# Mikata-Project/adcraft

Measured on AMD Instinct MI355X. Metric: env-steps/sec (envs×keywords auctions/s), higher is better.
Workload: dtype i32 cents + f32 (Philox4x32-7 u32); 1 GPU; cfg2: 4096 envs x 256 keywords per GPU, IMPLICIT keywords, mean_volume 128, cvr 0.8, no_vol_prob 0.0, drift False, budget non-binding, 60-step episodes with auto-reset; envs_per_gpu=4096, keywords=256, parallelism=env-sharded x1, collective=none (single GPU), weak_scaling_reference=also.cfg4.value of the N=1 --full line (same per-GPU shard as the N>1 runs)

## Files before the change

adcraft_amd/_ffi.py:

```python
import ctypes as C
import os

from . import build as _build

ADC_OK, ADC_EINVAL, ADC_EHIP, ADC_ENOMEM, ADC_ESTATE, ADC_ETYPE, ADC_ERCCL = 0, -1, -2, -3, -4, -5, -6
MODEL_IMPLICIT, MODEL_EXPLICIT, MODEL_IMPLICIT_GENERAL = 0, 1, 2
P_VOL_MEAN, P_VOL_STD, P_A, P_B, P_BCTR, P_SCTR, P_REV_MEAN, P_REV_STD, P_COUNT = range(9)
(BUF_PARAMS, BUF_BIDS, BUF_BUDGET, BUF_IMPRESSIONS, BUF_CLICKS, BUF_CONVERSIONS, BUF_COST, BUF_REVENUE, BUF_REWARD,
 BUF_CUM_PROFIT, BUF_DAYS, BUF_TERMINATED, BUF_TRUNCATED, BUF_METRIC_PROFIT, BUF_METRIC_SCALARS, BUF_FLAT_OBS,
 BUF_ROLLOUT_ACTION, BUF_ROLLOUT_LOGP, BUF_ROLLOUT_VALUE, BUF_ROLLOUT_REWARD, BUF_ROLLOUT_TERMINATED, BUF_ROLLOUT_TRUNCATED,
 BUF_ROLLOUT_OBS) = range(23)
MLP_TANH, MLP_RELU = 0, 1
ES_CENTERED_RANK, ES_RAW = 0, 1
ES_ADAM, ES_SGD = 0, 1
ROLLOUT_OBS = 1
PG_ADAM, PG_SGD = 0, 1
TD3_ADAM, TD3_SGD = 0, 1
PBT_PG, PBT_TD3 = 0, 1


class EngineError(RuntimeError):
    pass


# ... 194 lines not shown
        "adc_engine_metrics_reset": ([vp], C.c_int),
        "adc_engine_metrics_read": ([vp, vp, vp], C.c_int),
        "adc_engine_ideal_profit": ([vp, C.c_int, vp, C.c_int, vp], C.c_int),
        "adc_bid_curves_from_samples": ([C.c_int, vp, i32, vp, i32, vp, vp], C.c_int),
        "adc_engine_metrics_akncp_ncp": ([vp, f64, vp, vp], C.c_int),
        "adc_engine_bid_curves_contenders": ([vp, vp, vp, C.POINTER(i32)], C.c_int),
        "adc_engine_outcomes_replay": ([vp, i32, i32, vp, f32, i64, vp, vp, vp, vp, C.POINTER(i64), vp], C.c_int),
        "adc_engine_outcomes_replay_tape": ([vp, i32, vp, f32, C.POINTER(Tape), i64, vp, vp, vp, vp, C.POINTER(i64), vp], C.c_int),
        "adc_nth_price_auction": ([C.c_int, f64, vp, i32, i32, i32, i32, C.POINTER(i32), vp, vp], C.c_int),
        "adc_sigmoid": ([f64, f64, f64], f64),
        "adc_clamp": ([f64, f64, f64], f64),
        "adc_threshold_sigmoid": ([f64, f64, f64, f64], f64),
        "adc_sum_f64": ([vp, i64], f64),
        "adc_count_true": ([vp, i64], i64),
        "adc_nonneg_int_normal": ([f64, f64, u64, u64], u64),
        "adc_binomial": ([u64, f64, u64, u64], u64),
        "adc_cost_create": ([f64, i64, u64, u64, vp], C.c_int),
        "adc_auction_word_intervals": ([f32, f32, f32, f32, vp], C.c_int),
        "adc_auction_word_brackets": ([f32, f32, f32, f32, vp], C.c_int),
        "adc_check_win_brackets": ([i64, vp, vp, vp, vp, vp, vp, vp], i64),
        "adc_lower_bound_v_host": ([i64, vp, vp, vp, vp, vp], C.c_int),
        "adc_lower_bound_v_bisect_host": ([i64, vp, vp, vp, vp, vp], C.c_int),
        "adc_win_intervals_host": ([i64, vp, vp, vp, vp, i32, vp, vp], C.c_int),
        "adc_sample_random_keyword": ([C.c_uint64, C.c_uint32, C.c_uint32, vp], C.c_int),
        "adc_interp_act_host": ([f32, i32, f32, i32, C.c_double, C.c_double, C.c_double, vp, i32, i32, vp, vp, i32, vp, vp,
                                 C.c_double, vp, vp, vp, vp, vp], C.c_int),
        "adc_interp_key_host": ([f32], C.c_double),
        "adc_engine_mlp_init": ([vp, C.POINTER(MLPConfig), vp], C.c_int),
        "adc_engine_mlp_set_layer": ([vp, i32, i32, vp, vp], C.c_int),
        "adc_engine_mlp_set_norm": ([vp, vp, vp], C.c_int),
        "adc_engine_mlp_set_log_std": ([vp, vp], C.c_int),
        "adc_engine_mlp_set_deterministic": ([vp, i32], C.c_int),
        "adc_engine_mlp_act": ([vp, f32, vp], C.c_int),
        "adc_engine_mlp_step": ([vp, f32], C.c_int),
        "adc_engine_mlp_last": ([vp, vp, vp, vp, vp, vp], C.c_int),
        "adc_engine_mlp_bootstrap_value": ([vp, vp], C.c_int),
        "adc_engine_mlp_agent_state": ([vp, vp, vp], C.c_int),
        "adc_engine_rollout_enable": ([vp, i32, i32], C.c_int),
        "adc_engine_rollout_reset": ([vp], C.c_int),
        "adc_engine_rollout_fetch": ([vp, C.POINTER(i32), vp, vp, vp, vp, vp, vp, vp], C.c_int),
        "adc_engine_mlp_population": ([vp, i32, vp], C.c_int),
        "adc_engine_mlp_set_member_layer": ([vp, i32, i32, vp, vp], C.c_int),
        "adc_engine_mlp_param_count": ([vp, C.POINTER(i64)], C.c_int),
        "adc_engine_mlp_get_params": ([vp, vp], C.c_int),
        "adc_engine_mlp_get_member_params": ([vp, i32, vp], C.c_int),
        "adc_engine_mlp_learners": ([vp, i32], C.c_int),
# ... 171 lines not shown
```

adcraft_amd/build.py:

```python
import os
import subprocess
import sys

HERE = os.path.dirname(os.path.abspath(__file__))
ROOT = os.path.dirname(HERE)
SRC_DIR = os.path.join(HERE, "csrc")
LIB_DIR = os.path.join(HERE, "lib")
LIB = os.path.join(LIB_DIR, "libadcraft_hip.so")
SOURCES = ["adc_engine.hip", "adc_shims.cpp"]
HEADERS = ["adc_law.h", "adc_interp.h", "adc_mlp.h", "adc_es.h", "adc_pg.h", "adc_td3.h", "adc_pbt.h", "adc_norm.h", "adc_rew_norm.h", "adc_td3_norm.h", os.path.join(ROOT, "include", "adcraft_engine.h")] + sorted(
    os.path.join("parts", f) for f in os.listdir(os.path.join(SRC_DIR, "parts")) if f.endswith(".inc"))
HIPCC = os.environ.get("HIPCC", "/opt/rocm/bin/hipcc")
FLAGS = ["--offload-arch=gfx950", "-O3", "-std=c++17", "-fPIC", "-shared", "-fvisibility=hidden",
         "-ffp-contract=off", "-fno-fast-math", "-fhip-fp32-correctly-rounded-divide-sqrt",
         "-Wall", "-Wno-unused-function"]


def _deps():
    out = [os.path.join(SRC_DIR, s) for s in SOURCES]
    out += [h if os.path.isabs(h) else os.path.join(SRC_DIR, h) for h in HEADERS]
    return [p for p in out if os.path.exists(p)]


def source_hash():
    import hashlib
    h = hashlib.sha256()
    for p in sorted(_deps()):
        h.update(os.path.relpath(p, ROOT).encode() + b"\0")
        with open(p, "rb") as f:
            h.update(f.read())
    return h.hexdigest()[:16]


# ... 60 lines not shown
```

adcraft_amd/csrc/adc_engine.hip:

```cpp
#include <hip/hip_runtime.h>

#include <algorithm>
#include <chrono>
#include <type_traits>
#include <cmath>
#include <cstdio>
#include <cstdlib>
#include <cstring>
#include <new>
#include <string>
#include <vector>

#include "../../include/adcraft_engine.h"
#include "adc_law.h"
#include "adc_interp.h"
#include "adc_mlp.h"
#include "adc_es.h"
#include "adc_pg.h"
#include "adc_td3.h"
#include "adc_pbt.h"
#include "adc_norm.h"
#include "adc_rew_norm.h"
#include "adc_td3_norm.h"

#define ADC_EXPORT extern "C" __attribute__((visibility("default")))

namespace adck {
#include "parts/common.inc"
#include "parts/kernel_fast.inc"
#include "parts/kernel_sparse.inc"
#include "parts/kernel_exact_rows.inc"
#include "parts/kernel_click_walk.inc"
#include "parts/kernel_exact_serial.inc"
#include "parts/kernel_explicit_fast.inc"
#include "parts/kernels_misc.inc"
#include "parts/kernels_policy.inc"
#include "parts/kernel_explicit_curves.inc"
// ... 23 lines not shown
```

adcraft_amd/csrc/adc_shims.cpp:

```cpp
#include <algorithm>
#include <cmath>
#include <cstdint>
#include <thread>
#include <vector>

#include "../../include/adcraft_engine.h"
#include "adc_law.h"
#include "adc_interp.h"
#include "adc_mlp.h"
#include "adc_es.h"
#include "adc_pg.h"
#include "adc_td3.h"
#include "adc_pbt.h"
#include "adc_norm.h"
#include "adc_rew_norm.h"
#include "adc_td3_norm.h"

#define ADC_EXPORT extern "C" __attribute__((visibility("default")))

ADC_EXPORT double adc_sigmoid(double x, double s, double t) { return 1.0 / (1.0 + std::exp(-s * (x - t))); }

ADC_EXPORT double adc_clamp(double x, double lo, double hi) { return x < lo ? lo : (x > hi ? hi : x); }

ADC_EXPORT double adc_threshold_sigmoid(double p, double impression_thresh, double impression_bid_intercept,
                                        double impression_slope)
{
    const double halver = 2.0 + 1e-10;
    const double thresh = adc_clamp(halver * impression_thresh, 0.0, 1.0) / halver;
    const double r = adc_sigmoid(p, impression_slope, impression_bid_intercept);
    return adc_clamp((1.0 + 2.0 * thresh) * r - thresh, 0.0, 1.0);
// ... 161 lines not shown
    if (n < 0 || (n > 0 && (!bid_c || !cost_loc || !cost_scale || !buyside_ctr || !out4))) return ADC_EINVAL;
    const adc::LogTableEntry *table = host_log_table();
    shim_parallel_for(n, [=](int64_t i0, int64_t i1) {
        for (int64_t i = i0; i < i1; ++i) {
            const adc::AuctionLaw law = adc::make_auction_law(buyside_ctr[i]);
            const uint64_t t_click = adc::bernoulli_threshold(buyside_ctr[i]);
            uint32_t w_lo, w_hi;
            int stage = 0;
            if (bisect) {
                bool a = false, b = false;
                w_lo = adc::lower_bound_v_bisect(1 - bid_c[i], cost_loc[i], cost_scale[i], table, &a);
                w_hi = adc::lower_bound_v_bisect(bid_c[i], cost_loc[i], cost_scale[i], table, &b);
                stage = (a || b) ? 1 : 0;
            } else {
                adc::lower_bound_pair(bid_c[i], cost_loc[i], cost_scale[i], table, w_lo, w_hi, stage);
            }
            const adc::WinIntervals r = adc::win_intervals_of_bounds(w_lo, w_hi, t_click, law);
            uint32_t *o = out4 + 4 * i;
            o[0] = r.c_lo; o[1] = r.c_w; o[2] = r.n_lo; o[3] = r.n_w;
            if (stage_out) stage_out[i] = (uint8_t)stage;
        }
    });
    return ADC_OK;
}

ADC_EXPORT int adc_sample_random_keyword(uint64_t key, uint32_t keyword, uint32_t serial, float *out8)
{
    if (!out8) return ADC_EINVAL;
    adc::generate_explicit_keyword(key, keyword, serial, out8);
    return ADC_OK;
}

ADC_EXPORT int adc_explicit_curve_host(uint64_t key, uint32_t tick, int32_t keyword, int32_t n_samples, float impression_thresh, float a,
                                       float b, const double *bid_grid, int32_t n_bids, double *ir_out, double *cpc_out, double *z_mid2_out)
{
    if (n_samples <= 0 || n_samples > (1 << 20) || keyword < 0 || n_bids < 0 || (n_bids > 0 && (!bid_grid || !ir_out || !cpc_out)))
        return ADC_EINVAL;
    std::vector<float> z((size_t)n_samples);
    for (int32_t i = 0; i < n_samples; i += 4) {
        const adc::U4 w = adc::draw(key, (uint32_t)(i / 4), adc::ST_METRIC, (uint32_t)keyword, tick);
        const uint32_t ws[4] = {w.x, w.y, w.z, w.w};
        for (int j = 0; j < 4 && i + j < n_samples; ++j) z[(size_t)(i + j)] = adc::normal_from_word(ws[j]);
    }
    std::sort(z.begin(), z.end());
    const float z_lo = z[(size_t)((n_samples - 1) / 2)], z_hi = z[(size_t)(n_samples / 2)];
    if (z_mid2_out) { z_mid2_out[0] = z_lo; z_mid2_out[1] = z_hi; }
// ... 842 lines not shown
```

adcraft_amd/csrc/parts/common.inc:

```

thread_local std::string g_err;

int fail(int code, const std::string &msg)
{
    g_err = msg;
    return code;
}

#define HIP_TRY(expr)                                                                                     \
    do {                                                                                                  \
        hipError_t _e = (expr);                                                                           \
        if (_e != hipSuccess) {                                                                           \
            return fail(_e == hipErrorOutOfMemory ? ADC_ENOMEM : ADC_EHIP,                                \
                        std::string(#expr) + ": " + hipGetErrorString(_e));                               \
        }                                                                                                 \
    } while (0)

constexpr int kFastBlock = 256;
constexpr int kChunk = 16;
constexpr int kWave = 64;
constexpr int kProfileRing = 2048;
constexpr int kProfileMarks = 4;

#ifdef ADC_EXP_TIMING
__device__ unsigned long long g_dbg[16];
__device__ unsigned long long g_fdbg[256][8];
#define FDBG_T() __builtin_amdgcn_s_memtime()
#define FDBG_ADD(i, x) fdbg[i] += (x)
#else
#define FDBG_T() 0ull
#define FDBG_ADD(i, x) (void)0
#endif

struct RestState {
    long long R;
    double r_d;
    int row;
    int flags;
    long long pc;
};

struct View {
    int N, K, model, max_days;
    int NP;
    double loss_threshold;
    float drift_vol, drift_ctr, drift_cvr;
    int drift_on;
    float imp_thresh;
    int auto_reset;
    int metrics_on;
    int max_bidders, num_winners;
    float participation_rate;
    float *params;
    uint64_t *key;
// ... 265 lines not shown
```

adcraft_amd/csrc/parts/host_api.inc:

```
struct adc_engine {
    adc_config cfg;
    View v;
    hipStream_t stream = nullptr;
    float *d_bids = nullptr, *d_budget = nullptr;
    unsigned char *d_out_block = nullptr, *h_out_block = nullptr;
    size_t out_block_bytes = 0, out_off[10] = {0};
    float *h_act_block = nullptr;
    std::vector<void *> allocs;
    bool have_reset = false;
    int last_step = 0;
    int *h_binding = nullptr;
    size_t rest_table_count = 0;
    size_t click_rec_count = 0;
    bool in_capture = false;
    bool h_binding_off = false;
    bool fail_lazy_alloc = false;
    hipStream_t gstream[4] = {nullptr, nullptr, nullptr, nullptr};
    hipEvent_t ev_fork = nullptr, ev_join[4] = {nullptr, nullptr, nullptr, nullptr};
    int *d_counters = nullptr;
    int last_groups = 1;
    bool api_since_step = true;
    bool needs_fork = true;
    bool groups_pending = false;
    bool stream_exposed = false;
// ... 3572 lines not shown
    while (days > 0) {
        if ((rc = one_day(e, policy, budget))) return rc;
        days -= 1;
    }
    return ADC_OK;
}

#ifdef ADC_EXP_TIMING
extern "C" __attribute__((visibility("default"))) int adc_debug_read(unsigned long long *out, int reset)
{
    hipDeviceSynchronize();
    hipMemcpyFromSymbol(out, HIP_SYMBOL(g_dbg), sizeof(unsigned long long) * 16);
    static unsigned long long rows[256][8];
    hipMemcpyFromSymbol(rows, HIP_SYMBOL(g_fdbg), sizeof(rows));
    for (int i = 0; i < 8; ++i) { out[8 + i] = 0; for (int r = 0; r < 256; ++r) out[8 + i] += rows[r][i]; }
    if (reset) {
        unsigned long long z[16] = {0};
        hipMemcpyToSymbol(HIP_SYMBOL(g_dbg), z, sizeof(z));
        std::memset(rows, 0, sizeof(rows));
        hipMemcpyToSymbol(HIP_SYMBOL(g_fdbg), rows, sizeof(rows));
    }
    return 0;
}
#endif
```

adcraft_amd/csrc/parts/kernel_fast.inc:

```
constexpr int kQueueCap = 128;
constexpr int kDenseVolumePerKeyword = 24;

struct alignas(16) KwLawA {
    unsigned int m_click, t_conv;
    float loc, scale;
};
struct alignas(16) KwLawB {
    float mu, sd;
    union {
        struct {
            unsigned int t_click;
            int bid_c;
        } d;
        adc::KwHalf conv;
    };
};
union alignas(16) KwWin {
    adc::WinIntervals iv;
    struct { unsigned int m_noclick, pad0, pad1, pad2; } d;
};

constexpr int kClkShift = 21, kConvShift = 42;
static_assert(adc::kVolumeMax < (1 << kClkShift), "three counts of up to kVolumeMax must fit 21 bits each");

struct FastShared {
    union {
        struct {
            unsigned int tag[kFastBlock / kWave][kQueueCap];
            unsigned int word[kFastBlock / kWave][kQueueCap];
        } queue;
        struct {
            unsigned int volw[kFastBlock];
            int wave_tot[kFastBlock / kWave], wave_vol[kFastBlock / kWave], wave_live[kFastBlock / kWave];
        };
    };
    KwWin win[kFastBlock];
    KwLawA law_a[kFastBlock];
    KwLawB law_b[kFastBlock];
    unsigned long long a_cnt[kFastBlock], a_cost[kFastBlock], a_rev[kFastBlock];
    adc::LogTableEntry logtab[adc::kLogTableIntervals];
    float normtab[adc::kNormTableEntries + 1];
    int off[kFastBlock + 1];
    int vol[kFastBlock];
};
template <bool LISTS>
struct FastListing {
    unsigned int row_count[adc::kTimesteps];
    int jcut[kFastBlock];
    unsigned int price_cut;
};
template <>
struct FastListing<false> {};
static_assert(sizeof(FastShared) + sizeof(FastListing<true>) <= 25 * 1280, "the listing variant must allow 5 workgroups per CU too");
static_assert(kFastBlock == adc::kLogTableIntervals, "one table entry per lane is copied in phase 1");
static_assert(sizeof(FastShared) <= 25 * 1280, "FastShared must allow 5 workgroups per CU");

__device__ __forceinline__ float normal_tab_nodes(uint32_t w, const float *nodes)
{
    const uint32_t t = ((w >> 7) & 0x00FFFFFEu) | 1u;
    const uint32_t bits = __float_as_uint((float)t);
    const uint32_t i = (bits >> 18) - (127u << 5);
    const float a = nodes[i], b = nodes[i + 1];
    const float z = adc::fma32((b - a) * 3.814697265625e-06f, (float)(bits & 0x0003FFFFu), a);
    return __uint_as_float(__float_as_uint(z) | (~w & 0x80000000u));
}

struct FastRaw {
    float vol_mean, vol_std, bctr, sctr, loc, scale, mu, sd, bid;
    uint64_t key;
    uint32_t tick;
    bool drift, skip, emit;
};

template <bool NARROW, bool LISTS = false>
__global__ __launch_bounds__(kFastBlock, 5) void k_step_implicit_fast(View v, const float *__restrict__ bids, int tile_kw_arg, int tiles_per_wg)
{
    __shared__ FastShared sh;
    [[maybe_unused]] __shared__ FastListing<LISTS> ls;
    const int tile_kw = NARROW ? tile_kw_arg : kFastBlock;
    const int tiles = (v.K + tile_kw - 1) / tile_kw;
    const int tid = threadIdx.x;
    const int lane = tid & 63, wv = tid >> 6;
    [[maybe_unused]] unsigned long long fdbg[8] = {0, 0, 0, 0, 0, 0, 0, 0};

    auto load_tile = [&](int tile_index) {
        FastRaw r{};
        const int env = tile_index / tiles;
        const int k = (tile_index - env * tiles) * tile_kw + tid;
        r.key = v.key[env];
        r.tick = v.tick[env];
        r.drift = v.drift_on && v.drift_pending[env];
        const int hint = v.exact_hint[env];
        r.skip = (hint & ~4) == 2;
        r.emit = LISTS && hint == 1 && v.click_rec != nullptr;
        if (tid < tile_kw && k < v.K && !r.skip) {
            r.vol_mean = param_at(v, ADC_P_VOL_MEAN, env, k);
            r.vol_std = param_at(v, ADC_P_VOL_STD, env, k);
            r.bctr = param_at(v, ADC_P_BCTR, env, k);
            r.sctr = param_at(v, ADC_P_SCTR, env, k);
            r.loc = param_at(v, ADC_P_A, env, k);
            r.scale = param_at(v, ADC_P_B, env, k);
            r.mu = param_at(v, ADC_P_REV_MEAN, env, k);
            r.sd = param_at(v, ADC_P_REV_STD, env, k);
            r.bid = bids[(size_t)env * v.K + k];
        }
        return r;
    };

    const int n_tiles = v.N * tiles;
    const int tile_first = blockIdx.x * tiles_per_wg, tile_last = min(tile_first + tiles_per_wg, n_tiles);
    sh.logtab[tid] = g_log_table[tid];
    for (int i = tid; i <= adc::kNormTableEntries; i += kFastBlock) sh.normtab[i] = g_norm_nodes[i];
    FastRaw next = load_tile(tile_first);

  for (int tile_index = tile_first; tile_index < tile_last; ++tile_index) {
    const FastRaw raw = next;
    if (tile_index + 1 < tile_last) next = load_tile(tile_index + 1);
    if (raw.skip) continue;
    const int env = tile_index / tiles;
    const int tile = tile_index - env * tiles;
    const int k = tile * tile_kw + tid;
    const bool valid = tid < tile_kw && k < v.K;
    const uint64_t key = raw.key;
    const uint32_t tick = raw.tick;
    const uint32_t kw_base = (uint32_t)(tile * tile_kw);
    if (LISTS && raw.emit && tid == 0) v.click_tick[env] = tick + 1u;
    if constexpr (LISTS) { if (raw.emit && !NARROW && tid < adc::kTimesteps) ls.row_count[tid] = 0u; }
    [[maybe_unused]] const unsigned long long t_start = FDBG_T();

    if (tid < (tile_kw + 3) / 4) {
        const adc::U4 w = adc::draw(key, 0u, adc::ST_VOL, (kw_base >> 2) + (uint32_t)tid, tick);
        *reinterpret_cast<uint4 *>(&sh.volw[4 * tid]) = make_uint4(w.x, w.y, w.z, w.w);
    }
    float vol_mean = raw.vol_mean, bctr = raw.bctr, sctr = raw.sctr;
    const float vol_std = raw.vol_std, loc = raw.loc, scale = raw.scale, mu = raw.mu, sd = raw.sd, bid = raw.bid;
    if (valid && raw.drift && drift_keyword(v, env, key, tick - 1u, k, vol_mean, vol_std, bctr, sctr)) {
        param_at(v, ADC_P_VOL_MEAN, env, k) = vol_mean;
        param_at(v, ADC_P_BCTR, env, k) = bctr;
        param_at(v, ADC_P_SCTR, env, k) = sctr;
    }
    sh.a_cnt[tid] = sh.a_cost[tid] = sh.a_rev[tid] = 0ull;
    __syncthreads();
    int V = 0;
    if (valid) {
        float x = adc::fma32(vol_std, normal_tab_nodes(sh.volw[tid], sh.normtab), vol_mean);
        x = x > 0.0f ? x : 0.0f;
        x = x < (float)adc::kVolumeMax ? x : (float)adc::kVolumeMax;
        const float t = __builtin_truncf(x);
        V = (int)t + ((x - t) >= 0.5f ? 1 : 0);
    }
    sh.vol[tid] = V;
    if constexpr (LISTS) {
        if (raw.emit) {
            const int rows = (int)v.click_row_hint[env], s = V / adc::kTimesteps;
            ls.jcut[tid] = rows >= adc::kTimesteps - 1 ? 0x7FFFFFFF : V - (adc::kTimesteps - 1) * s + rows * s;
            if (tid == 0) ls.price_cut = v.click_price_hint[env];
        }
    }
    {
        const int vsum = wave_sum_i32(V);
        const int live = (int)__popcll(__builtin_amdgcn_ballot_w64(V > 0));
        if (lane == 0) { sh.wave_vol[wv] = vsum; sh.wave_live[wv] = live; }
    }
    __syncthreads();
    int tile_volume = 0, tile_live = 0;
#pragma unroll
    for (int i = 0; i < kFastBlock / kWave; ++i) { tile_volume += sh.wave_vol[i]; tile_live += sh.wave_live[i]; }
    const bool dense = tile_volume >= kDenseVolumePerKeyword * tile_live;
    const int chunk_shift = tile_volume >= 32 * kFastBlock ? 4 : tile_volume >= 16 * kFastBlock ? 3 : 2;
    const int chunk = 1 << chunk_shift;
    const int nch = V >> chunk_shift;
    const int incl = wave_scan_i32(nch);
    if (lane == 63) sh.wave_tot[wv] = incl;
    [[maybe_unused]] const unsigned long long t_law = FDBG_T();
    if (V > 0) {
        const uint64_t t_click = adc::bernoulli_threshold(bctr);
        const adc::AuctionLaw law = adc::make_auction_law(bctr);
        const int bid_c = (int)adc::bid_to_cents(bid);
        sh.law_a[tid] = KwLawA{law.m_click, adc::saturate_threshold(adc::bernoulli_threshold(sctr)), loc, scale};
        KwLawB lb;
        lb.mu = mu;
        lb.sd = sd;
        if (dense) {
            lb.conv = adc::philox_kw_half(adc::ST_CONV, kw_base + (uint32_t)tid, (uint32_t)key);
            sh.win[tid].iv = adc::win_intervals(bid_c, loc, scale, t_click, law, sh.logtab);
        } else {
            lb.d.t_click = law.t32;
            lb.d.bid_c = bid_c;
            sh.win[tid].d.m_noclick = law.m_noclick;
        }
        sh.law_b[tid] = lb;
    }
    FDBG_ADD(1, FDBG_T() - t_law);
    __syncthreads();
    int wave_base = 0, total = 0;
#pragma unroll
    for (int i = 0; i < kFastBlock / kWave; ++i) {
        const int t = sh.wave_tot[i];
        if (i < wv) wave_base += t;
        total += t;
    }
    __syncthreads();
    sh.off[tid] = wave_base + incl - nch;
    if (tid == 0) sh.off[kFastBlock] = total;
    __syncthreads();
    [[maybe_unused]] const unsigned long long t_p2 = FDBG_T();
    FDBG_ADD(0, t_p2 - t_start);

    const int wq = __builtin_amdgcn_readfirstlane(wv);
    unsigned int *const qtag = sh.queue.tag[wq];
    unsigned int *const qword = sh.queue.word[wq];
    unsigned int qtail = 0;

    auto resolve_click = [&](bool direct) {
        const uint2 ent = make_uint2(qtag[lane], qword[lane]);
        const unsigned int uu = ent.x >> 24;
        unsigned int acc_off = uu * (unsigned int)sizeof(unsigned long long);
        asm volatile("" : "+v"(acc_off));
        unsigned long long *const acc = (unsigned long long *)((char *)sh.a_cnt + acc_off);
        const KwLawA ka = sh.law_a[uu];
        const KwLawB kb = sh.law_b[uu];
        unsigned int price = ent.y;
        if (!direct) {
            unsigned int vv = adc::mulhi32(ent.y, ka.m_click);
            vv = vv < 0x00FFFFFFu ? vv : 0x00FFFFFFu;
            price = (unsigned int)adc::competitor_cents_from_v(vv, ka.loc, ka.scale, sh.logtab);
        }
        const adc::U4 w2 = direct ? adc::draw(key, ent.x & 0x00FFFFFFu, adc::ST_CONV, kw_base + uu, tick)
                                  : adc::draw_kw(key, ent.x & 0x00FFFFFFu, kb.conv, tick);
        const bool conv = adc::bernoulli32(w2.x, ka.t_conv);
        unsigned long long cnt = 1ull << kClkShift;
        if (conv) {
            float x = adc::fma32(kb.sd, normal_tab_nodes(w2.y, sh.normtab), kb.mu);
            x = x > 0.01f ? x : 0.01f;
            atomicAdd(acc + 2 * kFastBlock, (unsigned long long)(unsigned int)adc::money_to_cents(x));
            cnt |= 1ull << kConvShift;
        }
        atomicAdd(acc, cnt);
        atomicAdd(acc + kFastBlock, (unsigned long long)price);
        if constexpr (LISTS) { if (raw.emit) {
            const int j = (int)(ent.x & 0x00FFFFFFu);
            if (j < ls.jcut[uu] || price <= ls.price_cut) {
                const int V = sh.vol[uu];
                const int s = V / adc::kTimesteps, first = V - (adc::kTimesteps - 1) * s;
                int row = 0, jc = j;
                if (j >= first) {
                    const int d = j - first;
                    int q = (int)((float)d * __builtin_amdgcn_rcpf((float)s));
                    q -= q * s > d ? 1 : 0;
                    q += (q + 1) * s <= d ? 1 : 0;
                    row = 1 + q;
                    jc = d - q * s;
                }
                const unsigned int slot = NARROW ? atomicAdd(&v.click_count[(size_t)env * adc::kTimesteps + row], 1u) : atomicAdd(&ls.row_count[row], 1u);
                if (slot < click_seg_cap(v, row))
                    v.click_rec[click_seg_offset(v, env, row) + slot] = make_uint2(((kw_base + uu) << 20) | (unsigned int)jc, price);
            }
        } }
    };
    auto drain = [&](bool direct) {
        if (qtail >= (unsigned int)kWave) {
            [[maybe_unused]] const unsigned long long tb = FDBG_T();
            __builtin_amdgcn_fence(__ATOMIC_ACQ_REL, "wavefront");
            __builtin_amdgcn_wave_barrier();
            resolve_click(direct);
            qtail -= kWave;
            if ((unsigned int)lane < qtail) { qtag[lane] = qtag[kWave + lane]; qword[lane] = qword[kWave + lane]; }
            FDBG_ADD(4, FDBG_T() - tb);
            FDBG_ADD(7, 1);
        }
    };
    auto push = [&](bool click, unsigned int tagj, unsigned int payload) {
        const unsigned long long m = __builtin_amdgcn_ballot_w64(click);
        const unsigned int rank = __builtin_amdgcn_mbcnt_hi((unsigned int)(m >> 32), __builtin_amdgcn_mbcnt_lo((unsigned int)m, 0u));
        if (click) { (qtag + qtail)[rank] = tagj; (qword + qtail)[rank] = payload; }
        qtail += __popcll(m);
    };
    auto run_item = [&](auto tail_tag, int u, int j0, int n) {
        constexpr bool TAIL = decltype(tail_tag)::value;
        const uint32_t kw = kw_base + (uint32_t)u;
        const unsigned int tagj0 = ((unsigned int)u << 24) | (unsigned int)j0;
        unsigned int imp = 0;
        if (dense) {
            adc::WinIntervals iv = sh.win[u].iv;
            if (n == 0) iv.c_w = iv.n_w = 0u;
            asm volatile("" : "+v"(iv.c_w), "+v"(iv.n_w));
            for (int i = 0; i < chunk; i += 4) {
                if (TAIL && __builtin_amdgcn_ballot_w64(i < n) == 0ull) break;
                const adc::U4 w = adc::draw(key, (uint32_t)(j0 + i) >> 2, adc::ST_AUCTION, kw, tick);
#pragma unroll
                for (int h = 0; h < 4; ++h) {
                    const uint32_t word = h == 0 ? w.x : h == 1 ? w.y : h == 2 ? w.z : w.w;
                    bool cw = (word - iv.c_lo) < iv.c_w;
                    bool nw = (word - iv.n_lo) < iv.n_w;
                    if (TAIL) { const bool active = i + h < n; cw = cw && active; nw = nw && active; }
                    add_lane_bit(imp, __builtin_amdgcn_ballot_w64(cw) | __builtin_amdgcn_ballot_w64(nw));
                    push(cw, tagj0 + (unsigned int)(i + h), word);
                    drain(false);
                }
            }
        }
        if (!dense) {
            const KwLawA ka = sh.law_a[u];
            const KwLawB kb = sh.law_b[u];
            const adc::AuctionLaw law{kb.d.t_click, ka.m_click, sh.win[u].d.m_noclick};
            const int bid_c = n > 0 ? kb.d.bid_c : 0;
            for (int i = 0; i < chunk; i += 4) {
                if (TAIL && __builtin_amdgcn_ballot_w64(i < n) == 0ull) break;
                const adc::U4 w = adc::draw(key, (uint32_t)(j0 + i) >> 2, adc::ST_AUCTION, kw, tick);
#pragma unroll
                for (int h = 0; h < 4; ++h) {
                    const uint32_t word = h == 0 ? w.x : h == 1 ? w.y : h == 2 ? w.z : w.w;
                    bool click_bit;
                    const int comp = adc::auction_outcome_unless_top_word(word, law, ka.loc, ka.scale, sh.logtab, click_bit);
                    bool win = adc::auction_wins(word, bid_c, comp);
                    if (TAIL) win = win && i + h < n;
                    imp += (unsigned int)win;
                    push(win && click_bit, tagj0 + (unsigned int)(i + h), (unsigned int)comp);
                    drain(true);
                }
            }
        }
        if (imp) atomicAdd(&sh.a_cnt[u], (unsigned long long)imp);
    };

    const int rounds = (total + kFastBlock - 1) / kFastBlock;
    {
        const int first = min(tid * rounds, total), last = min(first + rounds, total);
        int u = 0;
#pragma unroll
        for (int s = kFastBlock / 2; s > 0; s >>= 1)
            if (sh.off[u + s] <= first) u += s;
        int u_end = sh.off[u + 1];
        for (int r = 0; r < rounds; ++r) {
            const int item = first + r;
            const bool has = item < last;
            [[maybe_unused]] const unsigned long long t_item = FDBG_T();
            while (has && item >= u_end) { u += 1; u_end = sh.off[u + 1]; }
            const int j0 = has ? (item - sh.off[u]) << chunk_shift : 0;
            FDBG_ADD(2, FDBG_T() - t_item);
            run_item(std::false_type{}, u, j0, has ? chunk : 0);
        }
        if (__syncthreads_or((V & (chunk - 1)) != 0)) run_item(std::true_type{}, tid, (V >> chunk_shift) << chunk_shift, V & (chunk - 1));
    }
    __builtin_amdgcn_fence(__ATOMIC_ACQ_REL, "wavefront");
    __builtin_amdgcn_wave_barrier();
    if ((unsigned int)lane < qtail) resolve_click(!dense);
    [[maybe_unused]] const unsigned long long t_p3 = FDBG_T();
    FDBG_ADD(3, t_p3 - t_p2);
    __syncthreads();

    if constexpr (LISTS) { if (raw.emit && !NARROW && tid < adc::kTimesteps) v.click_count[(size_t)env * adc::kTimesteps + tid] = ls.row_count[tid]; }
    if (valid) {
        const size_t o = (size_t)env * v.K + k;
        const unsigned long long cnt = sh.a_cnt[tid];
        const long long my_cost = (long long)sh.a_cost[tid];
        const long long r = (long long)sh.a_rev[tid];
        const unsigned int cnt_lo = (unsigned int)cnt, cnt_hi = (unsigned int)(cnt >> 32);
        v.imp[o] = (int)(cnt_lo & 0x1FFFFFu);
        v.clk[o] = (int)(((cnt_lo >> 21) | (cnt_hi << 11)) & 0x1FFFFFu);
        v.conv[o] = (int)(cnt_hi >> 10);
        v.cost[o] = adc::cents_to_dollars_f32(my_cost);
        v.rev[o] = adc::cents_to_dollars_f32(r);
        if (v.metrics_on) metric_add(v, o, r - my_cost);
    }
    if (wv == 0) {
// ... 3 lines not shown
            const int u = lane + i * kWave;
            if (u < tile_kw && tile * tile_kw + u < v.K) {
                const long long cc = (long long)sh.a_cost[u];
                c += cc;
                p += (long long)sh.a_rev[u] - cc;
            }
        }
        c = wave_sum_i64(c);
        p = wave_sum_i64(p);
        if (lane == 0) {
            if (tiles == 1) { v.env_cost[env] = c; v.env_profit[env] = p; }
            else {
                atomicAdd((unsigned long long *)&v.env_cost[env], (unsigned long long)c);
                atomicAdd((unsigned long long *)&v.env_profit[env], (unsigned long long)p);
            }
        }
    }
    FDBG_ADD(5, FDBG_T() - t_p3);
    FDBG_ADD(6, 1);
    __syncthreads();
  }
#ifdef ADC_EXP_TIMING
    if (tid == 0) for (int i = 0; i < 8; ++i) atomicAdd(&g_fdbg[blockIdx.x & 255][i], fdbg[i]);
#endif
}

__device__ __forceinline__ void step_tail(const View &v, int env, uint32_t tick, bool implicit, long long profit_c, double reward_d)
{
    double reward, cum;
    if (implicit) {
        const long long cc = v.cum_cents[env] + profit_c;
        v.cum_cents[env] = cc;
        reward = (double)profit_c / 100.0;
        cum = (double)cc / 100.0;
    } else {
        reward = reward_d;
        cum = v.cum[env] + reward;
        v.cum[env] = cum;
    }
    const bool truncated = cum < -v.loss_threshold;
    const int day = v.day[env] + 1;
    const bool terminated = day >= v.max_days;
    v.reward[env] = reward;
    v.cum_profit[env] = cum;
    v.day_out[env] = day;
    v.term[env] = terminated;
// ... 19 lines not shown
```

include/adcraft_engine.h:

```cpp
#ifndef ADCRAFT_ENGINE_H
#define ADCRAFT_ENGINE_H

#include <stddef.h>
#include <stdint.h>

#ifdef __cplusplus
extern "C" {
#endif

#define ADC_ABI_VERSION 5
#define ADC_STREAM_REVISION 5

typedef enum adc_status {
    ADC_OK = 0,
    ADC_EINVAL = -1,
    ADC_EHIP = -2,
    ADC_ENOMEM = -3,
    ADC_ESTATE = -4,
    ADC_ETYPE = -5,
    ADC_ERCCL = -6
} adc_status;

typedef enum adc_model {
    ADC_MODEL_IMPLICIT = 0,
// ... 481 lines not shown
                                    int32_t *keyword, int32_t *timestep, double *cost, double *revenue, int64_t *count, int32_t *share_volume_k);

int adc_nth_price_auction(int device_id, double bid, const double *other_bids, int32_t n_auctions, int32_t n_bidders,
                          int32_t n, int32_t num_winners, int32_t *impressions, int32_t *placements, double *costs);

double adc_sigmoid(double x, double s, double t);
double adc_clamp(double x, double lo, double hi);
double adc_threshold_sigmoid(double p, double impression_thresh,
                             double impression_bid_intercept, double impression_slope);
double adc_sum_f64(const double *x, int64_t n);
int64_t adc_count_true(const uint8_t *x, int64_t n);
uint64_t adc_nonneg_int_normal(double mean, double std, uint64_t seed, uint64_t counter);
uint64_t adc_binomial(uint64_t n, double p, uint64_t seed, uint64_t counter);
int adc_cost_create(double x, int64_t n, uint64_t seed, uint64_t counter, double *out_n);
int adc_auction_word_intervals(float bid, float cost_loc, float cost_scale, float buyside_ctr, uint32_t *out4);
int adc_auction_word_brackets(float bid, float cost_loc, float cost_scale, float buyside_ctr, uint32_t *out8);
int64_t adc_check_win_brackets(int64_t n, const float *bid, const float *cost_loc, const float *cost_scale, const float *buyside_ctr,
                               const uint32_t *brackets8, int64_t *first_bad, double *ambiguous_words);
int adc_lower_bound_v_host(int64_t n, const int32_t *target_n, const float *loc_n, const float *scale_n, uint32_t *v_n, uint8_t *stage_n);
int adc_lower_bound_v_bisect_host(int64_t n, const int32_t *target_n, const float *loc_n, const float *scale_n, uint32_t *v_n,
                                  uint8_t *whole_range_n);
int adc_win_intervals_host(int64_t n, const int32_t *bid_cents_n, const float *cost_loc_n, const float *cost_scale_n,
                           const float *buyside_ctr_n, int32_t bisect, uint32_t *out4_n, uint8_t *stage_n);
int adc_sample_random_keyword(uint64_t key, uint32_t keyword, uint32_t serial, float *out8);
int adc_explicit_curve_host(uint64_t key, uint32_t tick, int32_t keyword, int32_t n_samples, float impression_thresh, float a, float b,
                            const double *bid_grid, int32_t n_bids, double *ir_out, double *cpc_out, double *z_mid2_out);
int adc_interp_act_host(float ave_rpc, int32_t num_rpc_obs, float ave_sctr, int32_t num_sctr_obs, double max_observed,
                        double profit_acquisition_threshold, double bid_step, const double *allowed_bids, int32_t n_bids,
                        int32_t n_clicks, const uint16_t *clicks_cent, const float *ave_clicks, int32_t n_cpc, const uint16_t *cpc_cent,
                        const double *ave_cpc, double u, double *margin_out, double *cost_out, double *bid_out, int32_t *index_out,
                        double *mass_out);
double adc_interp_key_host(float bid);
int adc_mlp_act_host(const adc_mlp_config *cfg, int32_t num_keywords, const float *obs_d, const float *const *policy_w,
                     const float *const *policy_b, const float *const *value_w, const float *const *value_b, const float *shift_d,
                     const float *scale_d, const float *log_std_a, const float *normals_a, uint64_t agent_key, uint32_t tick,
                     float budget_override, float *mean_a, float *log_std_out_a, float *action_a, float *logp, float *value,
                     float *bids_k, float *budget);
int adc_es_config_check(const adc_es_config *cfg, const char **message);
int adc_es_noise_host(uint64_t seed, uint32_t pair, uint32_t generation, int64_t p0, int64_t n, float *eps_n);
int adc_es_update_host(const adc_es_config *cfg, uint64_t seed, int32_t members, int64_t n_params, const double *fitness_m, int64_t generation,
                       float *theta_p, float *m_p, float *v_p, float *grad_p);
int adc_pg_config_check(const adc_pg_config *cfg, const char **message);
int adc_pg_gae_host(const adc_pg_config *cfg, int32_t days, int32_t num_envs, const float *reward_tn, const uint8_t *terminated_tn,
                    const uint8_t *truncated_tn, const float *value_tn, const float *bootstrap_n, float *adv_tn, float *ret_tn);
int adc_pg_param_count_host(const adc_mlp_config *mlp, int32_t num_keywords, int64_t *count);
int adc_pg_grad_host(const adc_mlp_config *mlp, int32_t num_keywords, const adc_pg_config *cfg, const float *theta_q, int64_t count,
// ... 38 lines not shown
```

Measured before the change: 6.578 billion keyword-steps/s.

## Schedule fast-kernel auction work per wave with separate tail-call pass

Reworks the fast auction kernel's work distribution. Remainder (tail) draws that do not fill a full chunk are now scheduled as a second pass of 4-wide calls, with a shared tail-keyword table and packed prefix scans, instead of a whole-block tail item. Work is also partitioned per wave, rotated by tile index, rather than per thread across the block. This aims to cut idle lanes and imbalance from partial chunks. It adds a host-side reference of the schedule, debug slot counters, and readfirstlane on key and tick, in exchange for more shared memory and a second loop pass.

```diff
diff --git a/adcraft_amd/_ffi.py b/adcraft_amd/_ffi.py
--- a/adcraft_amd/_ffi.py
+++ b/adcraft_amd/_ffi.py
@@ -240,6 +240,7 @@
         "adc_lower_bound_v_host": ([i64, vp, vp, vp, vp, vp], C.c_int),
         "adc_lower_bound_v_bisect_host": ([i64, vp, vp, vp, vp, vp], C.c_int),
         "adc_win_intervals_host": ([i64, vp, vp, vp, vp, i32, vp, vp], C.c_int),
+        "adc_fast_schedule_host": ([vp, i32, i32, vp, i64, vp, vp], i64),
         "adc_sample_random_keyword": ([C.c_uint64, C.c_uint32, C.c_uint32, vp], C.c_int),
         "adc_interp_act_host": ([f32, i32, f32, i32, C.c_double, C.c_double, C.c_double, vp, i32, i32, vp, vp, i32, vp, vp,
                                  C.c_double, vp, vp, vp, vp, vp], C.c_int),
diff --git a/adcraft_amd/build.py b/adcraft_amd/build.py
--- a/adcraft_amd/build.py
+++ b/adcraft_amd/build.py
@@ -8,7 +8,7 @@
 LIB_DIR = os.path.join(HERE, "lib")
 LIB = os.path.join(LIB_DIR, "libadcraft_hip.so")
 SOURCES = ["adc_engine.hip", "adc_shims.cpp"]
-HEADERS = ["adc_law.h", "adc_interp.h", "adc_mlp.h", "adc_es.h", "adc_pg.h", "adc_td3.h", "adc_pbt.h", "adc_norm.h", "adc_rew_norm.h", "adc_td3_norm.h", os.path.join(ROOT, "include", "adcraft_engine.h")] + sorted(
+HEADERS = ["adc_law.h", "adc_fast_schedule.h", "adc_interp.h", "adc_mlp.h", "adc_es.h", "adc_pg.h", "adc_td3.h", "adc_pbt.h", "adc_norm.h", "adc_rew_norm.h", "adc_td3_norm.h", os.path.join(ROOT, "include", "adcraft_engine.h")] + sorted(
     os.path.join("parts", f) for f in os.listdir(os.path.join(SRC_DIR, "parts")) if f.endswith(".inc"))
 HIPCC = os.environ.get("HIPCC", "/opt/rocm/bin/hipcc")
 FLAGS = ["--offload-arch=gfx950", "-O3", "-std=c++17", "-fPIC", "-shared", "-fvisibility=hidden",
diff --git a/adcraft_amd/csrc/adc_engine.hip b/adcraft_amd/csrc/adc_engine.hip
--- a/adcraft_amd/csrc/adc_engine.hip
+++ b/adcraft_amd/csrc/adc_engine.hip
@@ -13,6 +13,7 @@
 
 #include "../../include/adcraft_engine.h"
 #include "adc_law.h"
+#include "adc_fast_schedule.h"
 #include "adc_interp.h"
 #include "adc_mlp.h"
 #include "adc_es.h"
diff --git a/adcraft_amd/csrc/adc_fast_schedule.h b/adcraft_amd/csrc/adc_fast_schedule.h
--- /dev/null
+++ b/adcraft_amd/csrc/adc_fast_schedule.h
@@ -0,0 +1,51 @@
+#pragma once
+#include "adc_law.h"
+
+namespace adc {
+
+constexpr int kFastTileLanes = 256;
+constexpr int kFastWaveLanes = 64;
+constexpr int kFastTileWaves = kFastTileLanes / kFastWaveLanes;
+static_assert((kFastTileWaves & (kFastTileWaves - 1)) == 0, "fast_wave_part masks with kFastTileWaves - 1");
+constexpr int kFastCallShift = 2;
+constexpr int kDenseVolumePerKeyword = 24;
+
+ADC_HD bool fast_tile_dense(int tile_volume, int tile_live) { return tile_volume >= kDenseVolumePerKeyword * tile_live; }
+
+ADC_HD int fast_chunk_shift(int tile_volume)
+{
+    return tile_volume >= 32 * kFastTileLanes ? 4 : tile_volume >= 16 * kFastTileLanes ? 3 : 2;
+}
+
+ADC_HD int fast_full_items(int V, int chunk_shift) { return V >> chunk_shift; }
+ADC_HD int fast_tail_calls(int V, int chunk_shift) { return (V & ((1 << chunk_shift) - 1)) >> kFastCallShift; }
+ADC_HD int fast_tail_first(int V, int chunk_shift) { return (V >> chunk_shift) << chunk_shift; }
+ADC_HD int fast_partial_first(int V) { return (V >> kFastCallShift) << kFastCallShift; }
+ADC_HD int fast_partial_count(int V) { return V & ((1 << kFastCallShift) - 1); }
+constexpr int kFastTailCallsMax = 3;
+constexpr int kFastPackShift = 23;
+ADC_HD int fast_pack_counts(int full_items, int tail_calls) { return full_items | (tail_calls << kFastPackShift); }
+ADC_HD int fast_packed_items(int packed) { return packed & ((1 << kFastPackShift) - 1); }
+ADC_HD int fast_packed_calls(int packed) { return packed >> kFastPackShift; }
+ADC_HD int fast_calls_needed(int V) { return (V + (1 << kFastCallShift) - 1) >> kFastCallShift; }
+
+ADC_HD int fast_wave_part(int w, int tile_index) { return (w + tile_index) & (kFastTileWaves - 1); }
+ADC_HD int fast_wave_rounds(int total, int w)
+{
+    const int wave_rounds = (total + kFastWaveLanes - 1) / kFastWaveLanes;
+    return wave_rounds / kFastTileWaves + (w < wave_rounds % kFastTileWaves ? 1 : 0);
+}
+ADC_HD int fast_wave_base(int total, int w)
+{
+    const int wave_rounds = (total + kFastWaveLanes - 1) / kFastWaveLanes;
+    const int q = wave_rounds / kFastTileWaves, r = wave_rounds % kFastTileWaves;
+    return kFastWaveLanes * (w * q + (w < r ? w : r));
+}
+ADC_HD int fast_lane_first(int base, int rounds, int lane, int total)
+{
+    const int first = base + lane * rounds;
+    return first < total ? first : total;
+}
+ADC_HD bool fast_item_exists(int item, int total) { return item < total; }
+
+}
diff --git a/adcraft_amd/csrc/adc_shims.cpp b/adcraft_amd/csrc/adc_shims.cpp
--- a/adcraft_amd/csrc/adc_shims.cpp
+++ b/adcraft_amd/csrc/adc_shims.cpp
@@ -6,6 +6,7 @@
 
 #include "../../include/adcraft_engine.h"
 #include "adc_law.h"
+#include "adc_fast_schedule.h"
 #include "adc_interp.h"
 #include "adc_mlp.h"
 #include "adc_es.h"
@@ -213,6 +214,95 @@
         }
     });
     return ADC_OK;
+}
+
+ADC_EXPORT int64_t adc_fast_schedule_host(const int32_t *vol_k, int32_t tile_kw, int32_t tile_index, int32_t *slots7, int64_t cap, int64_t *totals2,
+                                          int32_t *info2)
+{
+    constexpr int B = adc::kFastTileLanes, WL = adc::kFastWaveLanes, NW = adc::kFastTileWaves;
+    if (!vol_k || tile_kw < 1 || tile_kw > B || tile_index < 0 || cap < 0 || (cap > 0 && !slots7)) return ADC_EINVAL;
+    int V[B];
+    int64_t volume = 0, needed = 0;
+    int live = 0;
+    for (int t = 0; t < B; ++t) {
+        V[t] = t < tile_kw ? vol_k[t] : 0;
+        if (V[t] < 0 || V[t] > adc::kVolumeMax) return ADC_EINVAL;
+        volume += V[t];
+        live += V[t] > 0;
+        needed += adc::fast_calls_needed(V[t]);
+    }
+    const int tile_volume = (int)volume;
+    const int chunk_shift = adc::fast_chunk_shift(tile_volume);
+    std::vector<int> off((size_t)B + 1), first_call((size_t)B);
+    std::vector<unsigned char> tail_kw((size_t)(adc::kFastTailCallsMax * B));
+    int total = 0, total2 = 0;
+    for (int w = 0; w < NW; ++w) {
+        int packed = 0;
+        for (int lane = 0; lane < WL; ++lane) {
+            const int t = w * WL + lane;
+            const int nch = adc::fast_full_items(V[t], chunk_shift), ntc = adc::fast_tail_calls(V[t], chunk_shift);
+            packed += adc::fast_pack_counts(nch, ntc);
+            off[(size_t)t] = total + adc::fast_packed_items(packed) - nch;
+            first_call[(size_t)t] = total2 + adc::fast_packed_calls(packed) - ntc;
+            for (int c = 0; c < adc::kFastTailCallsMax; ++c)
+                if (c < ntc) tail_kw[(size_t)(first_call[(size_t)t] + c)] = (unsigned char)t;
+        }
+        total += adc::fast_packed_items(packed);
+        total2 += adc::fast_packed_calls(packed);
+    }
+    off[(size_t)B] = total;
+    int64_t rows = 0, issued = 0;
+    auto emit = [&](int pass, int w, int r, int lane, int u, int j0, int n) {
+        if (rows < cap) {
+            int32_t *o = slots7 + 7 * rows;
+            o[0] = pass; o[1] = w; o[2] = r; o[3] = lane; o[4] = n > 0 ? u : -1; o[5] = n > 0 ? j0 : 0; o[6] = n;
+        }
+        rows += 1;
+    };
+    for (int pass = 0; pass < 2; ++pass) {
+        const int shift = pass == 0 ? chunk_shift : adc::kFastCallShift;
+        const int ptotal = pass == 0 ? total : total2;
+        for (int w = 0; w < NW; ++w) {
+            const int part = adc::fast_wave_part(w, tile_index);
+            const int rounds = adc::fast_wave_rounds(ptotal, part), base = adc::fast_wave_base(ptotal, part);
+            issued += (int64_t)rounds << (shift - adc::kFastCallShift);
+            for (int lane = 0; lane < WL; ++lane) {
+                const int first = adc::fast_lane_first(base, rounds, lane, ptotal);
+                int u = 0, u_end = 0;
+                if (pass == 0) {
+                    for (int s = B / 2; s > 0; s >>= 1)
+                        if (off[(size_t)(u + s)] <= first) u += s;
+                    u_end = off[(size_t)u + 1];
+                }
+                for (int r = 0; r < rounds; ++r) {
+                    const int item = first + r;
+                    const bool has = adc::fast_item_exists(item, ptotal);
+                    int j0 = 0;
+                    if (pass == 0) {
+                        while (has && item >= u_end) { u += 1; u_end = off[(size_t)u + 1]; }
+                        if (has) j0 = (item - off[(size_t)u]) << shift;
+                    } else if (has) {
+                        u = tail_kw[(size_t)item];
+                        j0 = adc::fast_tail_first(V[u], chunk_shift) + ((item - first_call[(size_t)u]) << shift);
+                    }
+                    emit(pass, w, r, lane, u, j0, has ? 1 << shift : 0);
+                }
+            }
+        }
+    }
+    for (int w = 0; w < NW; ++w) {
+        bool any = false;
+        for (int lane = 0; lane < WL; ++lane) any = any || adc::fast_partial_count(V[w * WL + lane]) != 0;
+        if (!any) continue;
+        issued += 1;
+        for (int lane = 0; lane < WL; ++lane) {
+            const int t = w * WL + lane;
+            emit(2, w, 0, lane, t, adc::fast_partial_first(V[t]), adc::fast_partial_count(V[t]));
+        }
+    }
+    if (totals2) { totals2[0] = issued; totals2[1] = needed; }
+    if (info2) { info2[0] = chunk_shift; info2[1] = adc::fast_tile_dense(tile_volume, live) ? 1 : 0; }
+    return rows;
 }
 
 ADC_EXPORT int adc_sample_random_keyword(uint64_t key, uint32_t keyword, uint32_t serial, float *out8)
diff --git a/adcraft_amd/csrc/parts/common.inc b/adcraft_amd/csrc/parts/common.inc
--- a/adcraft_amd/csrc/parts/common.inc
+++ b/adcraft_amd/csrc/parts/common.inc
@@ -27,9 +27,12 @@
 __device__ unsigned long long g_fdbg[256][8];
 #define FDBG_T() __builtin_amdgcn_s_memtime()
 #define FDBG_ADD(i, x) fdbg[i] += (x)
+__device__ unsigned long long g_fslots[256][2];
+#define FSLOT_ADD(i, x) fslots[i] += (x)
 #else
 #define FDBG_T() 0ull
 #define FDBG_ADD(i, x) (void)0
+#define FSLOT_ADD(i, x) (void)0
 #endif
 
 struct RestState {
diff --git a/adcraft_amd/csrc/parts/host_api.inc b/adcraft_amd/csrc/parts/host_api.inc
--- a/adcraft_amd/csrc/parts/host_api.inc
+++ b/adcraft_amd/csrc/parts/host_api.inc
@@ -3618,4 +3618,18 @@
     }
     return 0;
 }
+
+extern "C" __attribute__((visibility("default"))) int adc_debug_read_fast_slots(unsigned long long *out2, int reset)
+{
+    hipDeviceSynchronize();
+    static unsigned long long rows[256][2];
+    hipMemcpyFromSymbol(rows, HIP_SYMBOL(g_fslots), sizeof(rows));
+    out2[0] = out2[1] = 0;
+    for (int r = 0; r < 256; ++r) { out2[0] += rows[r][0]; out2[1] += rows[r][1]; }
+    if (reset) {
+        std::memset(rows, 0, sizeof(rows));
+        hipMemcpyToSymbol(HIP_SYMBOL(g_fslots), rows, sizeof(rows));
+    }
+    return 0;
+}
 #endif
diff --git a/adcraft_amd/csrc/parts/kernel_fast.inc b/adcraft_amd/csrc/parts/kernel_fast.inc
--- a/adcraft_amd/csrc/parts/kernel_fast.inc
+++ b/adcraft_amd/csrc/parts/kernel_fast.inc
@@ -1,5 +1,6 @@
 constexpr int kQueueCap = 128;
-constexpr int kDenseVolumePerKeyword = 24;
+constexpr int kDenseVolumePerKeyword = adc::kDenseVolumePerKeyword;
+static_assert(kFastBlock == adc::kFastTileLanes && kWave == adc::kFastWaveLanes, "adc_fast_schedule.h describes this workgroup");
 
 struct alignas(16) KwLawA {
     unsigned int m_click, t_conv;
@@ -21,6 +22,10 @@
 };
 
 constexpr int kClkShift = 21, kConvShift = 42;
+constexpr int kVolBits = 21;
+constexpr int kVolMask = (1 << kVolBits) - 1;
+constexpr int kTailCallsMax = adc::kFastTailCallsMax * kFastBlock;
+static_assert(adc::kVolumeMax <= kVolMask && kTailCallsMax < (1 << (31 - kVolBits)), "volume and tail-call prefix share a word");
 static_assert(adc::kVolumeMax < (1 << kClkShift), "three counts of up to kVolumeMax must fit 21 bits each");
 
 struct FastShared {
@@ -42,6 +47,7 @@
     float normtab[adc::kNormTableEntries + 1];
     int off[kFastBlock + 1];
     int vol[kFastBlock];
+    unsigned char tail_kw[kTailCallsMax];
 };
 template <bool LISTS>
 struct FastListing {
@@ -82,6 +88,7 @@
     const int tid = threadIdx.x;
     const int lane = tid & 63, wv = tid >> 6;
     [[maybe_unused]] unsigned long long fdbg[8] = {0, 0, 0, 0, 0, 0, 0, 0};
+    [[maybe_unused]] unsigned long long fslots[2] = {0, 0};
 
     auto load_tile = [&](int tile_index) {
         FastRaw r{};
@@ -121,8 +128,9 @@
     const int tile = tile_index - env * tiles;
     const int k = tile * tile_kw + tid;
     const bool valid = tid < tile_kw && k < v.K;
-    const uint64_t key = raw.key;
-    const uint32_t tick = raw.tick;
+    const uint64_t key = ((uint64_t)(uint32_t)__builtin_amdgcn_readfirstlane((int)(uint32_t)(raw.key >> 32)) << 32) |
+                         (uint32_t)__builtin_amdgcn_readfirstlane((int)(uint32_t)raw.key);
+    const uint32_t tick = (uint32_t)__builtin_amdgcn_readfirstlane((int)raw.tick);
     const uint32_t kw_base = (uint32_t)(tile * tile_kw);
     if (LISTS && raw.emit && tid == 0) v.click_tick[env] = tick + 1u;
     if constexpr (LISTS) { if (raw.emit && !NARROW && tid < adc::kTimesteps) ls.row_count[tid] = 0u; }
@@ -149,7 +157,6 @@
         const float t = __builtin_truncf(x);
         V = (int)t + ((x - t) >= 0.5f ? 1 : 0);
     }
-    sh.vol[tid] = V;
     if constexpr (LISTS) {
         if (raw.emit) {
             const int rows = (int)v.click_row_hint[env], s = V / adc::kTimesteps;
@@ -166,12 +173,13 @@
     int tile_volume = 0, tile_live = 0;
 #pragma unroll
     for (int i = 0; i < kFastBlock / kWave; ++i) { tile_volume += sh.wave_vol[i]; tile_live += sh.wave_live[i]; }
-    const bool dense = tile_volume >= kDenseVolumePerKeyword * tile_live;
-    const int chunk_shift = tile_volume >= 32 * kFastBlock ? 4 : tile_volume >= 16 * kFastBlock ? 3 : 2;
-    const int chunk = 1 << chunk_shift;
-    const int nch = V >> chunk_shift;
-    const int incl = wave_scan_i32(nch);
+    const bool dense = adc::fast_tile_dense(tile_volume, tile_live);
+    const int chunk_shift = adc::fast_chunk_shift(tile_volume);
+    const int nch = adc::fast_full_items(V, chunk_shift);
+    const int ntc = adc::fast_tail_calls(V, chunk_shift);
+    const int incl = wave_scan_i32(adc::fast_pack_counts(nch, ntc));
     if (lane == 63) sh.wave_tot[wv] = incl;
+    FSLOT_ADD(1, (unsigned long long)adc::fast_calls_needed(V));
     [[maybe_unused]] const unsigned long long t_law = FDBG_T();
     if (V > 0) {
         const uint64_t t_click = adc::bernoulli_threshold(bctr);
@@ -193,15 +201,23 @@
     }
     FDBG_ADD(1, FDBG_T() - t_law);
     __syncthreads();
-    int wave_base = 0, total = 0;
+    int wave_base = 0, total = 0, wave_base2 = 0, total2 = 0;
 #pragma unroll
     for (int i = 0; i < kFastBlock / kWave; ++i) {
         const int t = sh.wave_tot[i];
-        if (i < wv) wave_base += t;
-        total += t;
-    }
-    __syncthreads();
-    sh.off[tid] = wave_base + incl - nch;
+        if (i < wv) { wave_base += adc::fast_packed_items(t); wave_base2 += adc::fast_packed_calls(t); }
+        total += adc::fast_packed_items(t);
+        total2 += adc::fast_packed_calls(t);
+    }
+    __syncthreads();
+    sh.off[tid] = wave_base + adc::fast_packed_items(incl) - nch;
+    {
+        const int first_call = wave_base2 + adc::fast_packed_calls(incl) - ntc;
+        sh.vol[tid] = V | (first_call << kVolBits);
+#pragma unroll
+        for (int c = 0; c < adc::kFastTailCallsMax; ++c)
+            if (c < ntc) sh.tail_kw[first_call + c] = (unsigned char)tid;
+    }
     if (tid == 0) sh.off[kFastBlock] = total;
     __syncthreads();
     [[maybe_unused]] const unsigned long long t_p2 = FDBG_T();
@@ -241,7 +257,7 @@
         if constexpr (LISTS) { if (raw.emit) {
             const int j = (int)(ent.x & 0x00FFFFFFu);
             if (j < ls.jcut[uu] || price <= ls.price_cut) {
-                const int V = sh.vol[uu];
+                const int V = sh.vol[uu] & kVolMask;
                 const int s = V / adc::kTimesteps, first = V - (adc::kTimesteps - 1) * s;
                 int row = 0, jc = j;
                 if (j >= first) {
@@ -276,7 +292,7 @@
         if (click) { (qtag + qtail)[rank] = tagj; (qword + qtail)[rank] = payload; }
         qtail += __popcll(m);
     };
-    auto run_item = [&](auto tail_tag, int u, int j0, int n) {
+    auto run_item = [&](auto tail_tag, int u, int j0, int n, int calls4) {
         constexpr bool TAIL = decltype(tail_tag)::value;
         const uint32_t kw = kw_base + (uint32_t)u;
         const unsigned int tagj0 = ((unsigned int)u << 24) | (unsigned int)j0;
@@ -285,8 +301,9 @@
             adc::WinIntervals iv = sh.win[u].iv;
             if (n == 0) iv.c_w = iv.n_w = 0u;
             asm volatile("" : "+v"(iv.c_w), "+v"(iv.n_w));
-            for (int i = 0; i < chunk; i += 4) {
+            for (int i = 0; i < calls4; i += 4) {
                 if (TAIL && __builtin_amdgcn_ballot_w64(i < n) == 0ull) break;
+                FSLOT_ADD(0, 1ull);
                 const adc::U4 w = adc::draw(key, (uint32_t)(j0 + i) >> 2, adc::ST_AUCTION, kw, tick);
 #pragma unroll
                 for (int h = 0; h < 4; ++h) {
@@ -305,8 +322,9 @@
             const KwLawB kb = sh.law_b[u];
             const adc::AuctionLaw law{kb.d.t_click, ka.m_click, sh.win[u].d.m_noclick};
             const int bid_c = n > 0 ? kb.d.bid_c : 0;
-            for (int i = 0; i < chunk; i += 4) {
+            for (int i = 0; i < calls4; i += 4) {
                 if (TAIL && __builtin_amdgcn_ballot_w64(i < n) == 0ull) break;
+                FSLOT_ADD(0, 1ull);
                 const adc::U4 w = adc::draw(key, (uint32_t)(j0 + i) >> 2, adc::ST_AUCTION, kw, tick);
 #pragma unroll
                 for (int h = 0; h < 4; ++h) {
@@ -324,24 +342,42 @@
         if (imp) atomicAdd(&sh.a_cnt[u], (unsigned long long)imp);
     };
 
-    const int rounds = (total + kFastBlock - 1) / kFastBlock;
-    {
-        const int first = min(tid * rounds, total), last = min(first + rounds, total);
-        int u = 0;
-#pragma unroll
-        for (int s = kFastBlock / 2; s > 0; s >>= 1)
-            if (sh.off[u + s] <= first) u += s;
-        int u_end = sh.off[u + 1];
+#pragma nounroll
+    for (int pass = 0; pass < 2; ++pass) {
+        const int shift = pass == 0 ? chunk_shift : adc::kFastCallShift;
+        const int ptotal = pass == 0 ? total : total2;
+        const int part = adc::fast_wave_part(wq, tile_index);
+        const int rounds = __builtin_amdgcn_readfirstlane(adc::fast_wave_rounds(ptotal, part));
+        const int base = __builtin_amdgcn_readfirstlane(adc::fast_wave_base(ptotal, part));
+        if (rounds == 0) continue;
+        const int first = adc::fast_lane_first(base, rounds, lane, ptotal);
+        int u = 0, u_end = 0;
+        if (pass == 0) {
+#pragma unroll
+            for (int s = kFastBlock / 2; s > 0; s >>= 1)
+                if (sh.off[u + s] <= first) u += s;
+            u_end = sh.off[u + 1];
+        }
         for (int r = 0; r < rounds; ++r) {
             const int item = first + r;
-            const bool has = item < last;
+            const bool has = adc::fast_item_exists(item, ptotal);
             [[maybe_unused]] const unsigned long long t_item = FDBG_T();
-            while (has && item >= u_end) { u += 1; u_end = sh.off[u + 1]; }
-            const int j0 = has ? (item - sh.off[u]) << chunk_shift : 0;
+            int j0 = 0;
+            if (pass == 0) {
+                while (has && item >= u_end) { u += 1; u_end = sh.off[u + 1]; }
+                if (has) j0 = (item - sh.off[u]) << shift;
+            } else if (has) {
+                u = sh.tail_kw[item];
+                const int vw = sh.vol[u];
+                j0 = adc::fast_tail_first(vw & kVolMask, chunk_shift) + ((item - (int)((unsigned int)vw >> kVolBits)) << shift);
+            }
             FDBG_ADD(2, FDBG_T() - t_item);
-            run_item(std::false_type{}, u, j0, has ? chunk : 0);
-        }
-        if (__syncthreads_or((V & (chunk - 1)) != 0)) run_item(std::true_type{}, tid, (V >> chunk_shift) << chunk_shift, V & (chunk - 1));
+            run_item(std::false_type{}, u, j0, has ? 1 << shift : 0, 1 << shift);
+        }
+    }
+    if (__syncthreads_or(adc::fast_partial_count(V) != 0)) {
+        const int Vt = sh.vol[tid] & kVolMask;
+        run_item(std::true_type{}, tid, adc::fast_partial_first(Vt), adc::fast_partial_count(Vt), 1 << adc::kFastCallShift);
     }
     __builtin_amdgcn_fence(__ATOMIC_ACQ_REL, "wavefront");
     __builtin_amdgcn_wave_barrier();
@@ -391,6 +427,10 @@
   }
 #ifdef ADC_EXP_TIMING
     if (tid == 0) for (int i = 0; i < 8; ++i) atomicAdd(&g_fdbg[blockIdx.x & 255][i], fdbg[i]);
+    {
+        const unsigned long long needed = (unsigned long long)wave_sum_i64((long long)fslots[1]);
+        if (lane == 0) { atomicAdd(&g_fslots[blockIdx.x & 255][0], fslots[0]); atomicAdd(&g_fslots[blockIdx.x & 255][1], needed); }
+    }
 #endif
 }
 
diff --git a/include/adcraft_engine.h b/include/adcraft_engine.h
--- a/include/adcraft_engine.h
+++ b/include/adcraft_engine.h
@@ -527,6 +527,8 @@
                                   uint8_t *whole_range_n);
 int adc_win_intervals_host(int64_t n, const int32_t *bid_cents_n, const float *cost_loc_n, const float *cost_scale_n,
                            const float *buyside_ctr_n, int32_t bisect, uint32_t *out4_n, uint8_t *stage_n);
+int64_t adc_fast_schedule_host(const int32_t *vol_k, int32_t tile_kw, int32_t tile_index, int32_t *slots7, int64_t cap, int64_t *totals2,
+                               int32_t *info2);
 int adc_sample_random_keyword(uint64_t key, uint32_t keyword, uint32_t serial, float *out8);
 int adc_explicit_curve_host(uint64_t key, uint32_t tick, int32_t keyword, int32_t n_samples, float impression_thresh, float a, float b,
                             const double *bid_grid, int32_t n_bids, double *ir_out, double *cpc_out, double *z_mid2_out);
```

Measured after the change: 6.660 billion keyword-steps/s (median of 6 runs). +1.2%, better.
